# mapillary/OpenSfM

Measured on AMD Instinct MI355X. Metric: image-pairs matched/sec (+ BA LM-iters/sec, 5k cams / 500k pts), higher is better.
Workload: dtype i8 (exact int32 accumulate) + f64 RANSAC

## Files before the change

opensfm_amd/csrc/match.hip:

```cpp
#include <algorithm>
#include <cstdlib>
#include <type_traits>

#include "osfm_internal.h"

typedef int v4i __attribute__((ext_vector_type(4)));
typedef int v16i __attribute__((ext_vector_type(16)));

#ifdef OSFM_DBG_PHASES
__device__ unsigned long long g_phase[22];
#define OSFM_TICK(var) const unsigned long long var = wall_clock64();
#define OSFM_PHASE(i, t0, t1) if (threadIdx.x == 0) atomicAdd(&g_phase[i], (t1) - (t0));
extern "C" int osfm_dbg_phases(unsigned long long *out, int reset) {
  if (hipMemcpyFromSymbol(out, HIP_SYMBOL(g_phase), sizeof(g_phase)) != hipSuccess) return 1;
  if (reset) {
    unsigned long long z[22] = {};
    if (hipMemcpyToSymbol(HIP_SYMBOL(g_phase), z, sizeof(z)) != hipSuccess) return 1;
  }
  return 0;
}
#else
#define OSFM_TICK(var)
#define OSFM_PHASE(i, t0, t1)
#endif

namespace {

constexpr int kThreads = 256;
constexpr int kWaves = 4;
constexpr int kRT = 2;
constexpr int kNone = 0xFFFF;
constexpr int kCollisionD2 = 1 << 22;

__device__ __forceinline__ bool ratio_ok(int d1sq, int d2sq, double ratio) {
  if (ratio < 0.0) return (float)d1sq < (float)(-ratio) * (float)d2sq;
  const float f1 = sqrtf((float)d1sq), f2 = sqrtf((float)d2sq);
  return (double)f1 < ratio * (double)f2;
}

__device__ __forceinline__ long xcd_remap(long b, long n) {
  const long q = n >> 3, r = n & 7;
  const long xcd = b & 7, within = b >> 3;
  return (xcd < r ? xcd * (q + 1) : r * (q + 1) + (xcd - r) * q) + within;
}

struct MatchArgs {
  const int8_t *tiles;
  const int32_t *norms;
  const int32_t *hneg;
  const float *descf;
  const float *qerr;
  const int64_t *tile_off;
  const int32_t *counts;
  const int32_t *pairs;
  long n_pairs;
  double ratio;
  int symmetric;
  int query_second;
  int cap;
  int ncap;
  int32_t *out_counts;
  uint32_t *out_matches;
  int32_t *out_flags;
  long pad_tile;
  const uint32_t *bin;
  const float *seg;
  int32_t *tickets;
};
constexpr int kTicketStride = 32;

__device__ __forceinline__ void emit_matches(const MatchArgs &a, long p, int nC, const int *colBI,
                                             const unsigned short *rowres, int *misc, int tid, bool swap_halves) {
  const int lane = tid & 63, w = tid >> 6;
  int base = 0;
  for (int j0 = 0; j0 < nC; j0 += kThreads) {
    const int j = j0 + tid;
    bool m = false;
    int r = kNone;
    if (j < nC) {
      r = colBI[j];
      m = (r != kNone) && (!a.symmetric || rowres[r] == j);
    }
    const unsigned long long bal = __ballot(m);
    const int prefix = __popcll(bal & ((1ull << lane) - 1ull));
    if (lane == 0) misc[w] = __popcll(bal);
    __syncthreads();
    int woff = 0, total = 0;
#pragma unroll
    for (int w2 = 0; w2 < kWaves; ++w2) {
      const int cnt = misc[w2];
      woff += (w2 < w) ? cnt : 0;
      total += cnt;
    }
    if (m) {
      const int k = base + woff + prefix;
      if (k < a.cap) a.out_matches[p * a.cap + k] = swap_halves ? ((uint32_t)r | ((uint32_t)j << 16)) : ((uint32_t)j | ((uint32_t)r << 16));
    }
    base += total;
    __syncthreads();
  }
  if (tid == 0) a.out_counts[p] = base;
}

__device__ __forceinline__ int dot_rows8(const int8_t *tilesA, int rowA, const int8_t *tilesB, int rowB) {
  const int8_t *pa = tilesA + (long)(rowA >> 5) * OSFM_TILE_BYTES + (rowA & 31) * 16;
  const int8_t *pb = tilesB + (long)(rowB >> 5) * OSFM_TILE_BYTES + (rowB & 31) * 16;
  v4i av[8], bv[8];
#pragma unroll
  for (int q = 0; q < 8; ++q) {
    av[q] = *(const v4i *)(pa + q * 512);
    bv[q] = *(const v4i *)(pb + q * 512);
  }
  int s0 = 0, s1 = 0;
#pragma unroll
  for (int q = 0; q < 8; q += 2)
#pragma unroll
    for (int e = 0; e < 4; ++e) {
      s0 = __builtin_amdgcn_sdot4(av[q][e], bv[q][e], s0, false);
      s1 = __builtin_amdgcn_sdot4(av[q + 1][e], bv[q + 1][e], s1, false);
    }
  return s0 + s1;
}

template <class P>
__device__ __forceinline__ P *uniform_ptr(P *p) {
  const unsigned long long v = (unsigned long long)p;
  const unsigned lo = __builtin_amdgcn_readfirstlane((unsigned)v), hi = __builtin_amdgcn_readfirstlane((unsigned)(v >> 32));
  return (P *)(((unsigned long long)hi << 32) | lo);
}

__device__ __forceinline__ int wave_max(int v) {
#pragma unroll
  for (int m = 32; m >= 1; m >>= 1) v = max(v, __shfl_xor(v, m));
  return v;
}

__device__ __forceinline__ int row16_max(int x) {
  x = max(x, __builtin_amdgcn_update_dpp(x, x, 0xB1, 0xF, 0xF, false));
  x = max(x, __builtin_amdgcn_update_dpp(x, x, 0x4E, 0xF, 0xF, false));
  x = max(x, __builtin_amdgcn_update_dpp(x, x, 0x141, 0xF, 0xF, false));
  x = max(x, __builtin_amdgcn_update_dpp(x, x, 0x140, 0xF, 0xF, false));
  return x;
}

constexpr double kFqSlack = 8e-6;
__device__ __forceinline__ double fq_ratio(double ratio) { return ratio < 0.0 ? sqrt(-ratio) : ratio; }
__device__ __forceinline__ bool fq_surely_fails(int d0lo_sq, int d1hi_sq, double eps, double r) {
  const double D0lo = fmax(sqrt((double)max(d0lo_sq, 0)) - eps, 0.0) * (1.0 - kFqSlack);
  const double D1hi = (sqrt((double)max(d1hi_sq, 0)) + eps) * (1.0 + kFqSlack);
  return D0lo >= r * D1hi;
}
__device__ __forceinline__ bool fq_surely_passes(int d0hi_sq, int d1lo_sq, double eps, double r) {
  const double D0hi = (sqrt((double)max(d0hi_sq, 0)) + eps) * (1.0 + kFqSlack);
  const double D1lo = fmax(sqrt((double)max(d1lo_sq, 0)) - eps, 0.0) * (1.0 - kFqSlack);
  return D0hi < r * D1lo && D0hi < D1lo;
}
__device__ __forceinline__ float wave_minf(float v) {
#pragma unroll
  for (int m = 32; m >= 1; m >>= 1) v = fminf(v, __shfl_xor(v, m));
  return v;
}

constexpr int kCT4 = 8;
constexpr int kChunkCols4 = kCT4 * 32;
constexpr int kChunkBytes4 = kCT4 * OSFM_TILE_BYTES;

struct QueryPassShared {
  unsigned char *bbuf;
  int *hbuf;
};

template <bool GATHER, bool FQ, class Hooks>
__device__ __forceinline__ int query_pass(const QueryPassShared &sh, const int8_t *tilesQ, const int32_t *normQ, int nQ, int nslots,
                                          const unsigned short *qsel, const int8_t *tilesT, const int32_t *normT, const int32_t *hnegT,
                                          int nT, const int8_t *tiles_pad, const int32_t *hneg_pad, unsigned short *out, double ratio,
                                          int tid, const float *descQ, const float *descT, double eps, int *hit_word, int &any_hit,
                                          Hooks &&hooks) {
  asm volatile("" : "+v"(tid));
  asm volatile("" : "+s"(ratio));
  const int lane = tid & 63;
  const int w = __builtin_amdgcn_readfirstlane(tid >> 6);
  const int tT = (nT + 31) >> 5;
  const int tS = (nslots + 31) >> 5;
  const int nchunks = (tS + kCT4 - 1) / kCT4;
  const int nrb = (tT + kWaves * kRT - 1) / (kWaves * kRT);
  int flag = 0, hit = 0;

  auto dma_chunk = [&](int c) {
    unsigned char *dst = sh.bbuf + (c & 1) * kChunkBytes4;
#pragma unroll
    for (int q = 0; q < kCT4; ++q) {
      const int gt = c * kCT4 + q;
      const int8_t *src;
      if (GATHER) {
        const int slot = gt * 32 + (lane & 31);
        const int f = slot < nslots ? (int)qsel[slot] : 0;
        src = tilesQ + (long)(f >> 5) * OSFM_TILE_BYTES + w * 1024 + (lane >> 5) * 512 + (f & 31) * 16;
      } else {
        src = tilesQ + (long)(gt < tS ? gt : 0) * OSFM_TILE_BYTES + tid * 16;
      }
      __builtin_amdgcn_global_load_lds((const __attribute__((address_space(1))) void *)src,
                                       (__attribute__((address_space(3))) void *)(dst + q * OSFM_TILE_BYTES + w * 1024), 16, 0, 0);
    }
  };

  auto load_seeds = [&](int rb, int slot) {
    const int t = rb * (kWaves * kRT) + w * kRT;
    const int32_t *h0 = uniform_ptr((t < tT) ? hnegT + (long)t * 32 : hneg_pad);
    const int32_t *h1 = uniform_ptr((t + 1 < tT) ? hnegT + (long)(t + 1) * 32 : hneg_pad);
    const int32_t *hp = ((lane >> 5) ? h1 : h0) + (lane & 31);
    __builtin_amdgcn_global_load_lds((const __attribute__((address_space(1))) void *)hp,
                                     (__attribute__((address_space(3))) void *)(sh.hbuf + slot * 256 + w * 64), 4, 0, 0);
  };
  auto load_rows = [&](int rb, v4i (&af)[kRT][4], int rt) {
    const int t = rb * (kWaves * kRT) + w * kRT + rt;
    const auto *tp = (const __attribute__((address_space(1))) int8_t *)uniform_ptr((t < tT) ? tilesT + (long)t * OSFM_TILE_BYTES : tiles_pad);
#pragma unroll
    for (int ks = 0; ks < 4; ++ks) af[rt][ks] = *(const __attribute__((address_space(1))) v4i *)(tp + ks * 1024 + lane * 16);
  };
  auto load_targets = [&](int rb, v4i (&af)[kRT][4], int slot) {
    load_seeds(rb, slot);
    load_rows(rb, af, 0);
    load_rows(rb, af, 1);
  };
  v16i hn[kRT];
  auto read_seeds_rt = [&](int slot, int rt) {
#pragma unroll
    for (int g = 0; g < 4; ++g) {
      const v4i hv = *(const v4i *)(sh.hbuf + slot * 256 + w * 64 + rt * 32 + 8 * g + 4 * (lane >> 5));
      hn[rt][4 * g + 0] = hv[0];
      hn[rt][4 * g + 1] = hv[1];
      hn[rt][4 * g + 2] = hv[2];
      hn[rt][4 * g + 3] = hv[3];
    }
  };
  auto read_seeds = [&](int slot) {
    read_seeds_rt(slot, 0);
    read_seeds_rt(slot, 1);
  };

  int cb[kCT4], cs[kCT4], ci[kCT4];
  const unsigned char *bb = sh.bbuf;
  v4i bf[4];

#define OSFM_TREE_A(X, A, B)             \
  A = max(max(X[0], X[1]), X[2]);        \
  B = max(max(X[8], X[9]), X[10]);
#define OSFM_TREE_B(X, A, B)             \
  A = max(max(A, X[3]), X[4]);           \
  B = max(max(B, X[11]), X[12]);
#define OSFM_TREE_C(X, A, B)             \
  A = max(max(A, X[5]), X[6]);           \
  B = max(max(B, X[13]), X[14]);
// ... 25 lines not shown
        OSFM_TREE_A(C2, a0, b0)
        OSFM_TREE_B(C2, a0, b0)
        OSFM_TREE_C(C2, a0, b0)
        OSFM_TREE_D(C2, a0, b0, mp)
      } else {
        load_seeds(rbn, next_slot);
      }
      OSFM_PIN
      C2 = __builtin_amdgcn_mfma_i32_32x32x32_i8(af[1][0], bf[0], hn[1], 0, 0, 0);
      OSFM_PIN
      if (t == kCT4 - 1) {
        __builtin_amdgcn_s_waitcnt(0x0F70 | (2 * kRT * 4));
        read_seeds_rt(next_slot, 0);
      }
      bf[0] = *(const v4i *)(nb);
      if (t > 0) { OSFM_TREE_A(P2, a1, b1) }
      OSFM_PIN
      C1 = __builtin_amdgcn_mfma_i32_32x32x32_i8(af[0][1], bf[1], C1, 0, 0, 0);
      OSFM_PIN
      if (t > 0) { OSFM_TREE_B(P2, a1, b1) } else { load_rows(rbn, nxt, 0); }
      if (t == kCT4 - 1) read_seeds_rt(next_slot, 1);
      OSFM_PIN
      C2 = __builtin_amdgcn_mfma_i32_32x32x32_i8(af[1][1], bf[1], C2, 0, 0, 0);
      OSFM_PIN
      bf[1] = *(const v4i *)(nb + 1024);
      if (t > 0) { OSFM_TREE_C(P2, a1, b1) }
      OSFM_PIN
      C1 = __builtin_amdgcn_mfma_i32_32x32x32_i8(af[0][2], bf[2], C1, 0, 0, 0);
      OSFM_PIN
      if (t > 0) { OSFM_TREE_D(P2, a1, b1, m2) } else { load_rows(rbn, nxt, 1); }
      OSFM_PIN
      C2 = __builtin_amdgcn_mfma_i32_32x32x32_i8(af[1][2], bf[2], C2, 0, 0, 0);
      OSFM_PIN
      bf[2] = *(const v4i *)(nb + 2048);
      if (t > 0) {
        m2 = max(m2, mp);
        asm("v_med3_i32 %0, %1, %2, %3" : "=v"(cs[t - 1]) : "v"(cb[t - 1]), "v"(m2), "v"(cs[t - 1]));
      }
      OSFM_PIN
      C1 = __builtin_amdgcn_mfma_i32_32x32x32_i8(af[0][3], bf[3], C1, 0, 0, 0);
      OSFM_PIN
      if (t > 0)
        asm volatile("v_cmp_gt_i32 vcc, %1, %2\n\ts_nop 1\n\tv_cndmask_b32 %0, %0, %3, vcc" : "+v"(ci[t - 1]) : "v"(m2), "v"(cb[t - 1]), "v"(vrb) : "vcc");
      OSFM_PIN
      C2 = __builtin_amdgcn_mfma_i32_32x32x32_i8(af[1][3], bf[3], C2, 0, 0, 0);
      OSFM_PIN
      bf[3] = *(const v4i *)(nb + 3072);
      if (t > 0) cb[t - 1] = max(cb[t - 1], m2);
      OSFM_PIN
    }
    {
      v16i &Q1 = T[(2 * (kCT4 - 1)) % 3];
      v16i &Q2 = T[(2 * (kCT4 - 1) + 1) % 3];
      int a0, b0, a1, b1, m1, m2;
      OSFM_TREE_A(Q1, a0, b0)
      OSFM_TREE_B(Q1, a0, b0)
      OSFM_TREE_C(Q1, a0, b0)
      OSFM_TREE_D(Q1, a0, b0, m1)
      OSFM_TREE_A(Q2, a1, b1)
      OSFM_TREE_B(Q2, a1, b1)
      OSFM_TREE_C(Q2, a1, b1)
      OSFM_TREE_D(Q2, a1, b1, m2)
      m2 = max(m2, m1);
      asm("v_med3_i32 %0, %1, %2, %3" : "=v"(cs[kCT4 - 1]) : "v"(cb[kCT4 - 1]), "v"(m2), "v"(cs[kCT4 - 1]));
      ci[kCT4 - 1] = m2 > cb[kCT4 - 1] ? rb : ci[kCT4 - 1];
      cb[kCT4 - 1] = max(cb[kCT4 - 1], m2);
    }
  };

  auto load_norm = [&](int c) {
    const int slot = c * kChunkCols4 + tid;
    const int f = slot < nslots ? (GATHER ? (int)qsel[slot] : slot) : -1;
    return (f >= 0 && f < nQ) ? normQ[f] : OSFM_PAD_NORM;
  };
  dma_chunk(0);
  v4i afA[kRT][4], afB[kRT][4];
  load_targets(0, afA, 0);
  int myna_next = load_norm(0);
  hooks.cold_issue();
  __builtin_amdgcn_s_waitcnt(0x0F70);
  hooks.cold_done();
  read_seeds(0);
  int sidx = 0;

  for (int c = 0; c < nchunks; ++c) {
    const int myslot = c * kChunkCols4 + tid;
    const int myf = myslot < nslots ? (GATHER ? (int)qsel[myslot] : myslot) : -1;
    const int myna = myna_next;
    __builtin_amdgcn_s_waitcnt(0x0F70);
    __syncthreads();
    bb = sh.bbuf + (c & 1) * kChunkBytes4;
    const int t0 = kCT4 - min(kCT4, tS - c * kCT4);
#pragma unroll
    for (int ks = 0; ks < 4; ++ks) bf[ks] = *(const v4i *)(bb + ks * 1024 + lane * 16);
#pragma unroll
    for (int t = 0; t < kCT4; ++t) {
      cb[t] = INT_MIN;
      cs[t] = INT_MIN;
      ci[t] = 0;
    }

    auto one_step = [&](const v4i (&cur)[kRT][4], v4i (&nxt)[kRT][4], int rb) {
      const int rbn = (rb + 1 < nrb) ? rb + 1 : 0;
      const bool live = rb * (kWaves * kRT) + w * kRT < tT;
      const int nslot = (sidx + 1) & 1;
      if (live) {
        step(cur, nxt, rb, rbn, nslot, t0, bb - t0 * OSFM_TILE_BYTES);
      } else {
        load_targets(rbn, nxt, nslot);
        __builtin_amdgcn_s_waitcnt(0x0F70);
        read_seeds(nslot);
      }
      ++sidx;
    };
    OSFM_TICK(tk0)
    hooks.chunk(c);
    if (c + 1 < nchunks) dma_chunk(c + 1);
    int rb = 0;
    for (; rb + 1 < nrb; rb += 2) {
      one_step(afA, afB, rb);
      one_step(afB, afA, rb + 1);
    }
    if (rb < nrb) {
      one_step(afA, afB, rb);
#pragma unroll
      for (int rt = 0; rt < kRT; ++rt)
#pragma unroll
        for (int ks = 0; ks < 4; ++ks) afA[rt][ks] = afB[rt][ks];
    }

    OSFM_TICK(tk1)
    if (c + 1 < nchunks) myna_next = load_norm(c + 1);
    __syncthreads();
    OSFM_TICK(tk2)
    int *scr = (int *)(sh.bbuf + (c & 1) * kChunkBytes4);
    {
      const int part = w * 2 + (lane >> 5);
#pragma unroll
      for (int t = 0; t < kCT4; ++t) {
        const int qt = (t - t0) & (kCT4 - 1);
        scr[(part * 3 + 0) * kChunkCols4 + qt * 32 + (lane & 31)] = cb[t];
        scr[(part * 3 + 1) * kChunkCols4 + qt * 32 + (lane & 31)] = cs[t];
        scr[(part * 3 + 2) * kChunkCols4 + qt * 32 + (lane & 31)] = ci[t];
      }
    }
    __syncthreads();
    int b = INT_MIN, s2 = INT_MIN, id = 0;
#pragma unroll
    for (int part = 0; part < 2 * kWaves; ++part) {
      const int pb = scr[(part * 3 + 0) * kChunkCols4 + tid], ps = scr[(part * 3 + 1) * kChunkCols4 + tid];
      const int pi = scr[(part * 3 + 2) * kChunkCols4 + tid];
      s2 = max(max(s2, ps), min(b, pb));
      id = pb > b ? (pi * 8 + part) : id;
      b = max(b, pb);
    }
    __syncthreads();
    bool want = false;
    if (myf >= 0 && myf < nQ) {
      const int d1lo = max(myna - (2 * b + 1), 0), d2hi = myna - 2 * s2;
      if (FQ) {
        want = !fq_surely_fails(d1lo, d2hi, eps, fq_ratio(ratio));
      } else {
        if (d2hi >= kCollisionD2 && ratio >= 0.0) flag = 1;
        want = ratio_ok(d1lo, d2hi, ratio);
      }
#ifdef OSFM_DBG_NORECHECK
      want = false;
#endif
      if (!want) out[myf] = kNone;
    }
    unsigned long long pending = __ballot(want);
    unsigned long long redo = 0;
    OSFM_TICK(tk3)
#ifdef OSFM_DBG_PHASES
    if (tid == 0) atomicAdd(&g_phase[(GATHER ? 5 : 0) + 4], (unsigned long long)__popcll(pending));
#endif
    while (pending) {
      int srcs[4];
#pragma unroll
      for (int g = 0; g < 4; ++g) {
        srcs[g] = pending ? (int)__builtin_ctzll(pending) : -1;
        pending &= pending - 1;
      }
      const int g = lane >> 4, sl = lane & 15;
      const int src = g == 0 ? srcs[0] : g == 1 ? srcs[1] : g == 2 ? srcs[2] : srcs[3];
      const int ssrc = src < 0 ? 0 : src;
      const int qf = __shfl(myf, ssrc), qna = __shfl(myna, ssrc), qb = __shfl(b, ssrc), qs = __shfl(s2, ssrc), qid = __shfl(id, ssrc);
      const bool tie = (qs == qb);
      const int qrb = qid >> 3, qw = (qid >> 1) & 3, qh = qid & 1;
      const int row0 = (qrb * (kWaves * kRT) + qw * kRT) * 32 + (sl & 3) + 8 * (sl >> 2) + 4 * qh, row1 = row0 + 32;
      int k0 = INT_MIN, k1 = INT_MIN;
      if (src >= 0 && !tie) {
        const bool ok0 = row0 < nT, ok1 = row1 < nT;
        const int r0 = ok0 ? row0 : 0, r1 = ok1 ? row1 : 0;
        const int8_t *pa = tilesQ + (long)(qf >> 5) * OSFM_TILE_BYTES + (qf & 31) * 16;
        const int8_t *p0 = tilesT + (long)(r0 >> 5) * OSFM_TILE_BYTES + (r0 & 31) * 16;
        const int8_t *p1 = tilesT + (long)(r1 >> 5) * OSFM_TILE_BYTES + (r1 & 31) * 16;
        v4i av[8], bv0[8], bv1[8];
#pragma unroll
        for (int q = 0; q < 8; ++q) {
          av[q] = *(const v4i *)(pa + q * 512);
          bv0[q] = *(const v4i *)(p0 + q * 512);
          bv1[q] = *(const v4i *)(p1 + q * 512);
        }
        const int n0 = normT[r0], n1 = normT[r1];
        int s0 = 0, s1 = 0;
#pragma unroll
        for (int q = 0; q < 8; ++q)
#pragma unroll
          for (int e = 0; e < 4; ++e) {
            s0 = __builtin_amdgcn_sdot4(av[q][e], bv0[q][e], s0, false);
            s1 = __builtin_amdgcn_sdot4(av[q][e], bv1[q][e], s1, false);
          }
        if (ok0) k0 = (2 * s0 - n0) * 32 + (31 - sl);
        if (ok1) k1 = (2 * s1 - n1) * 32 + (15 - sl);
      }
      const int kmax = row16_max(max(k0, k1));
      const int ksec = row16_max(k0 == kmax ? k1 : (k1 == kmax ? k0 : max(k0, k1)));
      if (src >= 0) {
        bool full = tie;
        int win = kNone;
        if (!tie) {
          const int m1 = kmax >> 5, ord = 31 - (kmax & 31);
          const int jwin = (qrb * (kWaves * kRT) + qw * kRT + (ord >> 4)) * 32 + (ord & 3) + 8 * ((ord & 15) >> 2) + 4 * qh;
          const int m2 = ksec >> 5;
          const int sa = max(m2, 2 * qs), sb = max(m2, 2 * qs + 1);
          if (FQ) {
            const double r = fq_ratio(ratio);
            if (fq_surely_passes(qna - m1, qna - sb, eps, r))
              win = jwin;
            else if (!fq_surely_fails(qna - m1, qna - sa, eps, r))
              full = true;
          } else {
            const bool ra = ratio_ok(qna - m1, qna - sa, ratio), rbb = ratio_ok(qna - m1, qna - sb, ratio);
            if (ra == rbb)
              win = ra ? jwin : kNone;
            else
              full = true;
          }
        }
        if (sl == 0 && !full) out[qf] = (unsigned short)win;
        hit |= (!full && win != kNone);
        redo |= (full && sl == 0) ? (1ull << src) : 0ull;
      }
    }
    OSFM_TICK(tk4)
    OSFM_PHASE((GATHER ? 5 : 0) + 0, tk0, tk1)
    OSFM_PHASE((GATHER ? 5 : 0) + 1, tk1, tk2)
    OSFM_PHASE((GATHER ? 5 : 0) + 2, tk2, tk3)
    OSFM_PHASE((GATHER ? 5 : 0) + 3, tk3, tk4)
    {
      unsigned lo = (unsigned)redo, hi = (unsigned)(redo >> 32);
#pragma unroll
      for (int m = 32; m >= 16; m >>= 1) {
        lo |= (unsigned)__shfl_xor((int)lo, m);
        hi |= (unsigned)__shfl_xor((int)hi, m);
      }
      redo = ((unsigned long long)(unsigned)__builtin_amdgcn_readfirstlane((int)hi) << 32) | (unsigned)__builtin_amdgcn_readfirstlane((int)lo);
    }
    if (FQ) flag += __popcll(redo);
    while (FQ && redo) {
      const int src = __builtin_ctzll(redo);
      redo &= redo - 1;
      const int qf = __shfl(myf, src), qna = __shfl(myna, src), qs2 = __shfl(s2, src);
      const double T = (sqrt((double)max(qna - 2 * qs2, 0)) + 2.0 * eps) * (1.0 + 4.0 * kFqSlack) + 1e-6;
      const double T2 = T * T;
      const int vthr = T2 >= 2.0e9 ? INT_MIN : qna - (int)T2 - 1;
      const float *qrow = descQ + (long)qf * OSFM_DESC_DIM;
      float bd0 = INFINITY, bd1 = INFINITY;
      int bi0 = INT_MAX;
      for (int i = lane; i < nT; i += 64) {
        const int v = 2 * dot_rows8(tilesQ, qf, tilesT, i) - normT[i];
        if (v >= vthr) {
          const float sq = l2sqr_rows_f32(qrow, descT + (long)i * OSFM_DESC_DIM);
          const float d = ratio < 0.0 ? sq : sqrtf(sq);
          if (d < bd1) {
            if (bd0 > d) {
              bd1 = bd0;
              bd0 = d;
              bi0 = i;
            } else {
              bd1 = d;
            }
          }
        }
      }
      const float m = wave_minf(bd0);
      const int jwin = -wave_max(bd0 == m ? -bi0 : INT_MIN);
      const float sec = wave_minf(bi0 == jwin ? bd1 : bd0);
      const bool ok = ratio < 0.0 ? (m < (float)(-ratio) * sec) : ((double)m < ratio * (double)sec);
      if (lane == 0) out[qf] = (unsigned short)(ok ? jwin : kNone);
      hit |= ok;
    }
    while (!FQ && redo) {
      const int src = __builtin_ctzll(redo);
      redo &= redo - 1;
      const int qf = __shfl(myf, src), qna = __shfl(myna, src);
      int lv = INT_MIN, lj = INT_MAX, ls = INT_MIN;
      for (int i = lane; i < nT; i += 64) {
        const int v = 2 * dot_rows8(tilesQ, qf, tilesT, i) - normT[i];
        ls = max(ls, min(lv, v));
        if (v > lv) {
          lv = v;
          lj = i;
        }
      }
      const int m1 = wave_max(lv);
      const int jwin = -wave_max(lv == m1 ? -lj : INT_MIN);
      const int m2 = wave_max(lj == jwin ? ls : lv);
      const bool ok = ratio_ok(qna - m1, qna - m2, ratio);
      if (lane == 0) out[qf] = (unsigned short)(ok ? jwin : kNone);
      hit |= ok;
    }
  }
  if (hit) *hit_word = 1;
  __syncthreads();
  any_hit = *hit_word;
  return flag;
}

struct PairRange {
  long first;
  int len;
};
__device__ __forceinline__ PairRange pair_range(long n_pairs, int x) {
  const long q = n_pairs >> 3, r = n_pairs & 7;
  return PairRange{x < r ? x * (q + 1) : r * (q + 1) + (x - r) * q, (int)(q + (x < r ? 1 : 0))};
}
__device__ __forceinline__ int draw_pair(const MatchArgs &a, int xcd, int *hdr, bool have, int t) {
  for (int k = hdr[8]; k < 8; ++k) {
    const int x = (xcd + k) & 7;
    const PairRange r = pair_range(a.n_pairs, x);
    if (!have) t = atomicAdd(a.tickets + x * kTicketStride, 1);
    have = false;
    if (t < r.len) {
      hdr[8] = k;
      return (int)(r.first + t);
    }
  }
  hdr[8] = 8;
  return -1;
}
__device__ __forceinline__ void finish_pair_header(const MatchArgs &a, int *hdr) {
  const int img1 = hdr[1], img2 = hdr[2];
  const int n1 = a.counts[img1], n2 = a.counts[img2];
  const int o1 = (int)a.tile_off[img1], o2 = (int)a.tile_off[img2];
  hdr[3] = n1;
  hdr[4] = n2;
  hdr[5] = o1;
  hdr[6] = o2;
  hdr[7] = 1;
}
__device__ __forceinline__ void fetch_pair_header(const MatchArgs &a, int xcd, int *hdr) {
  const int p = draw_pair(a, xcd, hdr, false, 0);
  hdr[0] = p;
  hdr[7] = 1;
  if (p >= 0) {
    const int img1 = a.pairs[2 * (long)p], img2 = a.pairs[2 * (long)p + 1];
    hdr[1] = img1;
    hdr[2] = img2;
    finish_pair_header(a, hdr);
  }
}
struct NextPairFetch {
  const MatchArgs &a;
  int xcd;
  int *hdr;
  int tid;
  int t;
  __device__ __forceinline__ void cold_issue() {
    if (tid == 0) {
      const int k = hdr[8];
      t = k < 8 ? atomicAdd(a.tickets + ((xcd + k) & 7) * kTicketStride, 1) : 0;
    }
  }
  __device__ __forceinline__ void cold_done() {
    if (tid == 0) {
      hdr[0] = draw_pair(a, xcd, hdr, hdr[8] < 8, t);
      hdr[7] = 0;
    }
  }
  __device__ __forceinline__ void chunk(int c) {
    if (c > 1 || __builtin_amdgcn_readfirstlane(tid >> 6) != 0) return;
    const int pn = __builtin_amdgcn_readfirstlane(hdr[0]);
    if (pn < 0) return;
    if (c == 0) {
      if (tid < 2)
        __builtin_amdgcn_global_load_lds((const __attribute__((address_space(1))) void *)(a.pairs + 2 * (long)pn + tid),
                                         (__attribute__((address_space(3))) void *)(hdr + 1), 4, 0, 0);
    } else if (tid < 4) {
      const int img = hdr[1 + (tid & 1)];
      const int32_t *src = tid < 2 ? a.counts + img : (const int32_t *)(a.tile_off + img);
      __builtin_amdgcn_global_load_lds((const __attribute__((address_space(1))) void *)src,
                                       (__attribute__((address_space(3))) void *)(hdr + 3), 4, 0, 0);
      if (tid == 0) hdr[7] = 1;
    }
  }
};
struct NoFetch {
  __device__ __forceinline__ void cold_issue() {}
  __device__ __forceinline__ void cold_done() {}
  __device__ __forceinline__ void chunk(int) {}
};

__device__ __forceinline__ int fresh_tid(int wave) {
  int t = wave * 64 + (int)__builtin_amdgcn_mbcnt_hi(~0u, __builtin_amdgcn_mbcnt_lo(~0u, 0u));
  asm volatile("" : "+v"(t));
  return t;
}

template <bool FQ>
__global__ void __launch_bounds__(kThreads, 2) match_fused_kernel(MatchArgs a) {
  extern __shared__ __attribute__((aligned(16))) unsigned char smem[];
  QueryPassShared sh;
  sh.bbuf = smem;
  sh.hbuf = (int *)(smem + 2 * kChunkBytes4);
  int *misc = (int *)(smem + 2 * kChunkBytes4) + 2 * kChunkCols4;
  int *hdr = misc + 16;
  unsigned short *resA = (unsigned short *)(hdr + 16);
  unsigned short *resB = resA + a.ncap;
  unsigned short *cand = resB + a.ncap;

  const int xcd = blockIdx.x & 7;
  const int8_t *tiles_pad = a.tiles + a.pad_tile * OSFM_TILE_BYTES;
  const int32_t *hneg_pad = a.hneg + a.pad_tile * 32;
  OSFM_TICK(tw0)
#ifdef OSFM_DBG_PHASES
  unsigned long long t_prev = tw0;
#endif
  const int wave = __builtin_amdgcn_readfirstlane(threadIdx.x >> 6);
  if (threadIdx.x == 0) {
    hdr[8] = 0;
    fetch_pair_header(a, xcd, hdr);
  }
  __syncthreads();
  for (;;) {
  const int tid = fresh_tid(wave);
  const long p = __builtin_amdgcn_readfirstlane(hdr[0]);
  if (p < 0) break;
  if (__builtin_amdgcn_readfirstlane(hdr[7]) == 0) {
    __syncthreads();
    if (tid == 0) finish_pair_header(a, hdr);
    __syncthreads();
  }
  const int img1 = __builtin_amdgcn_readfirstlane(hdr[1]), img2 = __builtin_amdgcn_readfirstlane(hdr[2]);
  const int n1 = __builtin_amdgcn_readfirstlane(hdr[3]), n2 = __builtin_amdgcn_readfirstlane(hdr[4]);
  const long off1 = __builtin_amdgcn_readfirstlane(hdr[5]), off2 = __builtin_amdgcn_readfirstlane(hdr[6]);
  if (tid == 0) {
    misc[8] = 0;
    misc[9] = 0;
    misc[10] = 0;
  }
  __syncthreads();
  if (n1 < 2 || n2 < 2) {
    if (tid == 0) {
      a.out_counts[p] = 0;
      a.out_flags[p] = 0;
      fetch_pair_header(a, xcd, hdr);
    }
    __syncthreads();
#ifdef OSFM_DBG_PHASES
    {
      OSFM_TICK(te)
      OSFM_PHASE(19, t_prev, te)
      if (threadIdx.x == 0) atomicAdd(&g_phase[20], 1ull);
      t_prev = te;
    }
#endif
    continue;
  }
  const bool rows_second = a.symmetric || a.query_second;
  const int imgA = rows_second ? img2 : img1, imgB = rows_second ? img1 : img2;
  const int nA = rows_second ? n2 : n1, nB = rows_second ? n1 : n2;
  const long offA = rows_second ? off2 : off1, offB = rows_second ? off1 : off2;
  const int8_t *tilesA = a.tiles + offA * OSFM_TILE_BYTES;
  const int8_t *tilesB = a.tiles + offB * OSFM_TILE_BYTES;
  const int32_t *normA = a.norms + offA * 32;
  const int32_t *normB = a.norms + offB * 32;
  const int32_t *hnegA = a.hneg + offA * 32;
  const int32_t *hnegB = a.hneg + offB * 32;
  OSFM_TICK(tq0)
  const float *descA = FQ ? a.descf + offA * (long)(32 * OSFM_DESC_DIM) : nullptr;
  const float *descB = FQ ? a.descf + offB * (long)(32 * OSFM_DESC_DIM) : nullptr;
  const double eps = FQ ? (double)a.qerr[imgA] + (double)a.qerr[imgB] : 0.0;
  int any = 0;
  auto flush_flag = [&](int f) {
    if (FQ) {
      if ((fresh_tid(wave) & 63) == 0 && f) atomicAdd(&misc[8], f);
    } else if (f) {
      misc[8] = 1;
    }
  };
  int flag = query_pass<false, FQ>(sh, tilesA, normA, nA, nA, nullptr, tilesB, normB, hnegB, nB, tiles_pad, hneg_pad, resA, a.ratio, fresh_tid(wave),
                                   descA, descB, eps, misc + 9, any, NextPairFetch{a, xcd, hdr, fresh_tid(wave), 0});
  OSFM_TICK(tq1)
  OSFM_PHASE(10, tq0, tq1)
  if (a.symmetric && any) {
    const int tid = fresh_tid(wave), lane = tid & 63, w = tid >> 6;
    for (int j = tid; j < nB; j += kThreads) resB[j] = kNone;
    __syncthreads();
    for (int q = tid; q < nA; q += kThreads) {
      const int b = resA[q];
      if (b != kNone) resB[b] = 0;
    }
// ... 250 lines not shown
  const int nC = a.counts[imgC], nR = a.counts[imgR];
  if (nC < 2 || nR < 2) {
    if (tid == 0) a.out_counts[p] = 0;
    return;
  }
  const float *descC = a.descf + a.tile_off[imgC] * kFloatTileFloats;
  const float *descR = a.descf + a.tile_off[imgR] * kFloatTileFloats;
  float_direction(descC, nC, descR, nR, a.ratio, tid, stage, colBI, nullptr);
  if (a.symmetric) float_direction(descR, nR, descC, nC, a.ratio, tid, stage, nullptr, rowres);
  __syncthreads();
  emit_matches(a, p, nC, colBI, rowres, misc, tid, qs);
}

constexpr int kHamStageRows = 256;

__device__ void hamming_direction(const uint32_t *binQ, int nQ, const uint32_t *binT, int nT, double ratio, int tid, uint32_t *stage, int *res_int,
                                  unsigned short *res_u16) {
  for (int q0 = 0; q0 < nQ; q0 += kThreads) {
    const int q = q0 + tid;
    const bool live = q < nQ;
    uint4 qa[4];
#pragma unroll
    for (int k = 0; k < 4; ++k) qa[k] = live ? *(const uint4 *)(binQ + (size_t)q * 16 + 4 * k) : make_uint4(0u, 0u, 0u, 0u);
    int bd0 = 0x7fffffff, bd1 = 0x7fffffff, bi0 = kNone;
    for (int t0 = 0; t0 < nT; t0 += kHamStageRows) {
      const int nt = min(kHamStageRows, nT - t0);
      __syncthreads();
      for (int k = tid; k < nt * 4; k += kThreads) *(uint4 *)(stage + 4 * k) = *(const uint4 *)(binT + (size_t)t0 * 16 + 4 * k);
      __syncthreads();
      for (int t = 0; t < nt; ++t) {
        const uint4 *b = (const uint4 *)(stage + t * 16);
        int d = 0;
#pragma unroll
        for (int k = 0; k < 4; ++k) {
          const uint4 c = b[k];
          d += __popc(qa[k].x ^ c.x) + __popc(qa[k].y ^ c.y) + __popc(qa[k].z ^ c.z) + __popc(qa[k].w ^ c.w);
        }
        if (d < bd1) {
          if (bd0 > d) {
            bd1 = bd0;
            bd0 = d;
            bi0 = t0 + t;
          } else {
            bd1 = d;
          }
        }
      }
    }
    if (live) {
      const bool ok = (double)(float)bd0 < ratio * (double)(float)bd1;
      const int v = ok ? bi0 : kNone;
      if (res_int) res_int[q] = v;
      if (res_u16) res_u16[q] = (unsigned short)v;
    }
  }
}

__global__ void __launch_bounds__(kThreads) match_hamming_kernel(MatchArgs a) {
  extern __shared__ __attribute__((aligned(16))) unsigned char smem[];
  uint32_t *stage = (uint32_t *)smem;
  int *colBI = (int *)(stage + kHamStageRows * 16);
  unsigned short *rowres = (unsigned short *)(colBI + a.ncap);
  int *misc = (int *)(rowres + a.ncap);
  const int tid = threadIdx.x;
  const long p = blockIdx.x;
  if (tid == 0 && a.out_flags) a.out_flags[p] = 0;
  const bool qs = !a.symmetric && a.query_second;
  const int imgC = a.pairs[2 * p + (qs ? 1 : 0)], imgR = a.pairs[2 * p + (qs ? 0 : 1)];
  const int nC = a.counts[imgC], nR = a.counts[imgR];
  if (nC < 2 || nR < 2) {
    if (tid == 0) a.out_counts[p] = 0;
    return;
  }
  const uint32_t *binC = a.bin + a.tile_off[imgC] * (32 * 16);
  const uint32_t *binR = a.bin + a.tile_off[imgR] * (32 * 16);
  hamming_direction(binC, nC, binR, nR, a.ratio, tid, stage, colBI, nullptr);
  if (a.symmetric) hamming_direction(binR, nR, binC, nC, a.ratio, tid, stage, nullptr, rowres);
  __syncthreads();
  emit_matches(a, p, nC, colBI, rowres, misc, tid, qs);
}

}

size_t osfm_match_lds_bytes(int ncap) { return (size_t)2 * kChunkBytes4 + 2 * kChunkCols4 * 4 + 128 + (size_t)ncap * 6; }

static int ensure_kernel_attributes(int device) {
  static OsfmPerDeviceOnce once;
  return once.run(device, []() -> int {
    OSFM_HIP(hipFuncSetAttribute((const void *)match_fused_kernel<false>, hipFuncAttributeMaxDynamicSharedMemorySize, 160 * 1024));
    OSFM_HIP(hipFuncSetAttribute((const void *)match_fused_kernel<true>, hipFuncAttributeMaxDynamicSharedMemorySize, 160 * 1024));
    OSFM_HIP(hipFuncSetAttribute((const void *)match_exact_kernel, hipFuncAttributeMaxDynamicSharedMemorySize, 160 * 1024));
    OSFM_HIP(hipFuncSetAttribute((const void *)match_float_kernel, hipFuncAttributeMaxDynamicSharedMemorySize, 160 * 1024));
    OSFM_HIP(hipFuncSetAttribute((const void *)match_hamming_kernel, hipFuncAttributeMaxDynamicSharedMemorySize, 160 * 1024));
    return OSFM_OK;
  });
}

int osfm_launch_match(osfm_ctx *ctx, const osfm_store *store, const int32_t *d_pairs, int64_t n_pairs,
                      double ratio, int symmetric, int squared_ratio, int cap, int32_t *d_counts, uint32_t *d_matches,
                      int32_t *d_flags, bool exact_kernel, hipStream_t stream) {
  if (n_pairs == 0) return OSFM_OK;
  MatchArgs a;
  a.tiles = store->d_tiles;
  a.norms = store->d_norms;
  a.hneg = store->d_hneg;
  a.descf = store->d_descf;
  a.qerr = store->d_qerr;
  a.seg = store->d_seg;
  a.bin = store->d_bin;
  a.tile_off = store->d_tile_off;
  a.counts = store->d_counts;
  a.pairs = d_pairs;
  a.n_pairs = n_pairs;
  a.ratio = squared_ratio ? -(double)(float)(ratio * ratio) : ratio;
  a.symmetric = symmetric;
  a.query_second = squared_ratio && !symmetric;
  a.cap = cap;
  a.ncap = ((store->max_count + 127) / 128) * 128;
  if (a.ncap < 128) a.ncap = 128;
  a.out_counts = d_counts;
  a.out_matches = d_matches;
  a.out_flags = d_flags;
  a.pad_tile = store->tile_off[store->n_images];
  a.tickets = nullptr;
  OSFM_REQUIRE(a.ncap <= OSFM_MAX_FEATURES, OSFM_E_UNSUPPORTED, "more than %d features in an image", OSFM_MAX_FEATURES);
  OSFM_REQUIRE(n_pairs < (1ll << 31), OSFM_E_INVALID, "too many pairs in one launch");
  OSFM_TRY(ensure_kernel_attributes(ctx->device));
  const bool fused = !store->is_binary && !store->d_seg && !exact_kernel && (!store->is_float || store->quantised);
  unsigned resident = 0;
  if (fused) {
    OSFM_REQUIRE(a.pad_tile < (1ll << 31), OSFM_E_UNSUPPORTED, "too many tiles in the store");
    OSFM_REQUIRE(ctx->num_cus > 0, OSFM_E_INVALID, "the context knows no compute units");
    if (!ctx->d_match_tickets) OSFM_HIP(hipMalloc(&ctx->d_match_tickets, 8 * kTicketStride * sizeof(int32_t)));
    OSFM_HIP(hipMemsetAsync(ctx->d_match_tickets, 0, 8 * kTicketStride * sizeof(int32_t), stream));
    a.tickets = (int32_t *)ctx->d_match_tickets;
    resident = (unsigned)std::min<int64_t>(n_pairs, 2 * (int64_t)ctx->num_cus);
  }
  if (store->is_binary) {
    if (squared_ratio) a.ratio = ratio * ratio;
    if (exact_kernel && d_flags != nullptr) return OSFM_OK;
    const size_t lds = (size_t)kHamStageRows * 64 + (size_t)a.ncap * 6 + 64;
    hipLaunchKernelGGL(match_hamming_kernel, dim3((unsigned)n_pairs), dim3(kThreads), lds, stream, a);
  } else if (store->d_seg) {
    if (exact_kernel && d_flags != nullptr) return OSFM_OK;
    if (d_flags) OSFM_HIP(hipMemsetAsync(d_flags, 0, (size_t)n_pairs * sizeof(int32_t), stream));
    const size_t lds = (size_t)a.ncap * 6 + 64;
    hipLaunchKernelGGL(match_exact_kernel, dim3((unsigned)n_pairs), dim3(kThreads), lds, stream, a, 0);
  } else if (store->is_float) {
    if (exact_kernel && d_flags != nullptr) return OSFM_OK;
    if (!exact_kernel && store->quantised) {
      hipLaunchKernelGGL(match_fused_kernel<true>, dim3(resident), dim3(kThreads), osfm_match_lds_bytes(a.ncap), stream, a);
    } else {
      if (d_flags) OSFM_HIP(hipMemsetAsync(d_flags, 0, (size_t)n_pairs * sizeof(int32_t), stream));
      const size_t lds = (size_t)kFloatTileFloats * sizeof(float) + (size_t)a.ncap * 6 + 64;
      hipLaunchKernelGGL(match_float_kernel, dim3((unsigned)n_pairs), dim3(kThreads), lds, stream, a);
    }
  } else if (!exact_kernel) {
    hipLaunchKernelGGL(match_fused_kernel<false>, dim3(resident), dim3(kThreads), osfm_match_lds_bytes(a.ncap), stream, a);
  } else {
    const size_t lds = (size_t)a.ncap * 6 + 64;
    hipLaunchKernelGGL(match_exact_kernel, dim3((unsigned)n_pairs), dim3(kThreads), lds, stream, a, d_flags != nullptr ? 1 : 0);
  }
  OSFM_HIP(hipGetLastError());
  return OSFM_OK;
}
```

Baseline: 2.799 million.

## Batch ratio-test recheck candidates across chunks in LDS and spread over all waves

Instead of each wave immediately rechecking its own ambiguous queries after every chunk, candidates are appended to a block-wide LDS pending queue (with overflow into the scratch area) and flushed only once enough accumulate or at the last chunk. The flush spreads rounds of four candidates across all waves, double-buffers the gathers of target rows and query words, and broadcasts query words with ds_swizzle instead of loading them per lane. One barrier is dropped, and full fallback scans are deferred to a second pass marked by a redo bit. The intent is better load balance and latency hiding for the sparse recheck work, at the cost of added LDS, extra complexity, and longer liveness of pending entries.

After: 2.795 million. About the same (-0.1%).

```diff
diff --git a/opensfm_amd/csrc/match.hip b/opensfm_amd/csrc/match.hip
--- a/opensfm_amd/csrc/match.hip
+++ b/opensfm_amd/csrc/match.hip
@@ -8,13 +8,13 @@
 typedef int v16i __attribute__((ext_vector_type(16)));
 
 #ifdef OSFM_DBG_PHASES
-__device__ unsigned long long g_phase[22];
+__device__ unsigned long long g_phase[26];
 #define OSFM_TICK(var) const unsigned long long var = wall_clock64();
 #define OSFM_PHASE(i, t0, t1) if (threadIdx.x == 0) atomicAdd(&g_phase[i], (t1) - (t0));
 extern "C" int osfm_dbg_phases(unsigned long long *out, int reset) {
   if (hipMemcpyFromSymbol(out, HIP_SYMBOL(g_phase), sizeof(g_phase)) != hipSuccess) return 1;
   if (reset) {
-    unsigned long long z[22] = {};
+    unsigned long long z[26] = {};
     if (hipMemcpyToSymbol(HIP_SYMBOL(g_phase), z, sizeof(z)) != hipSuccess) return 1;
   }
   return 0;
@@ -168,7 +168,13 @@
 struct QueryPassShared {
   unsigned char *bbuf;
   int *hbuf;
+  int *pend;
+  int *pend_n;
 };
+constexpr int kPendFlush = 16;
+constexpr int kPendCap = kPendFlush;
+constexpr int kPendTie = 1 << 30;
+constexpr int kPendRedo = (int)0x80000000u;
 
 template <bool GATHER, bool FQ, class Hooks>
 __device__ __forceinline__ int query_pass(const QueryPassShared &sh, const int8_t *tilesQ, const int32_t *normQ, int nQ, int nslots,
@@ -360,6 +366,8 @@
   hooks.cold_done();
   read_seeds(0);
   int sidx = 0;
+  if (tid == 0) *sh.pend_n = 0;
+  int pend_done = 0;
 
   for (int c = 0; c < nchunks; ++c) {
     const int myslot = c * kChunkCols4 + tid;
@@ -400,6 +408,7 @@
       one_step(afB, afA, rb + 1);
     }
     if (rb < nrb) {
+      asm volatile("v_nop");
       one_step(afA, afB, rb);
 #pragma unroll
       for (int rt = 0; rt < kRT; ++rt)
@@ -432,7 +441,6 @@
       id = pb > b ? (pi * 8 + part) : id;
       b = max(b, pb);
     }
-    __syncthreads();
     bool want = false;
     if (myf >= 0 && myf < nQ) {
       const int d1lo = max(myna - (2 * b + 1), 0), d2hi = myna - 2 * s2;
@@ -447,149 +455,263 @@
 #endif
       if (!want) out[myf] = kNone;
     }
-    unsigned long long pending = __ballot(want);
-    unsigned long long redo = 0;
+    int *ovf = scr + 2 * kWaves * 3 * kChunkCols4;
+    {
+      const unsigned long long wb = __ballot(want);
+#ifdef OSFM_DBG_PHASES
+      if (tid == 0) atomicAdd(&g_phase[(GATHER ? 5 : 0) + 4], (unsigned long long)__popcll(wb));
+#endif
+      if (wb) {
+        int base = 0;
+        if (lane == 0) base = atomicAdd(sh.pend_n, (int)__popcll(wb));
+        base = __builtin_amdgcn_readfirstlane(base) - pend_done;
+        if (want) {
+          const int e = base + (int)__builtin_amdgcn_mbcnt_hi((unsigned)(wb >> 32), __builtin_amdgcn_mbcnt_lo((unsigned)wb, 0u));
+          int *ent = e < kPendCap ? sh.pend + 2 * e : ovf + 2 * (e - kPendCap);
+          ent[0] = myf | (id << 16) | (s2 == b ? kPendTie : 0);
+          ent[1] = s2;
+        }
+      }
+    }
+    __syncthreads();
     OSFM_TICK(tk3)
+    int npend;
+    {
+      auto *pn = (volatile __attribute__((address_space(3))) int *)sh.pend_n;
+      asm volatile("" : "+s"(pn));
+      npend = __builtin_amdgcn_readfirstlane(*pn) - pend_done;
+    }
+    if (npend > 0 && (npend >= kPendFlush || c + 1 == nchunks)) {
+      const int rounds = (npend + 3) >> 2;
 #ifdef OSFM_DBG_PHASES
-    if (tid == 0) atomicAdd(&g_phase[(GATHER ? 5 : 0) + 4], (unsigned long long)__popcll(pending));
+      if (tid == 0) {
+        atomicAdd(&g_phase[(GATHER ? 24 : 22)], 1ull);
+        atomicAdd(&g_phase[(GATHER ? 25 : 23)], (unsigned long long)rounds);
+      }
 #endif
-    while (pending) {
-      int srcs[4];
-#pragma unroll
-      for (int g = 0; g < 4; ++g) {
-        srcs[g] = pending ? (int)__builtin_ctzll(pending) : -1;
-        pending &= pending - 1;
-      }
-      const int g = lane >> 4, sl = lane & 15;
-      const int src = g == 0 ? srcs[0] : g == 1 ? srcs[1] : g == 2 ? srcs[2] : srcs[3];
-      const int ssrc = src < 0 ? 0 : src;
-      const int qf = __shfl(myf, ssrc), qna = __shfl(myna, ssrc), qb = __shfl(b, ssrc), qs = __shfl(s2, ssrc), qid = __shfl(id, ssrc);
-      const bool tie = (qs == qb);
-      const int qrb = qid >> 3, qw = (qid >> 1) & 3, qh = qid & 1;
-      const int row0 = (qrb * (kWaves * kRT) + qw * kRT) * 32 + (sl & 3) + 8 * (sl >> 2) + 4 * qh, row1 = row0 + 32;
-      int k0 = INT_MIN, k1 = INT_MIN;
-      if (src >= 0 && !tie) {
-        const bool ok0 = row0 < nT, ok1 = row1 < nT;
-        const int r0 = ok0 ? row0 : 0, r1 = ok1 ? row1 : 0;
-        const int8_t *pa = tilesQ + (long)(qf >> 5) * OSFM_TILE_BYTES + (qf & 31) * 16;
-        const int8_t *p0 = tilesT + (long)(r0 >> 5) * OSFM_TILE_BYTES + (r0 & 31) * 16;
-        const int8_t *p1 = tilesT + (long)(r1 >> 5) * OSFM_TILE_BYTES + (r1 & 31) * 16;
-        v4i av[8], bv0[8], bv1[8];
+      int fl = (int)__builtin_amdgcn_mbcnt_hi(~0u, __builtin_amdgcn_mbcnt_lo(~0u, 0u));
+      asm volatile("" : "+v"(fl));
+      const int g = fl >> 4, sl = fl & 15;
+      struct ReexamRound {
+        v4i t0[8], t1[8];
+        int qx, qy;
+        int n0, n1, qna;
+      };
+      typedef __attribute__((address_space(3))) int lds_int;
+      lds_int *pend3 = (lds_int *)sh.pend, *ovf3 = (lds_int *)ovf;
+      asm volatile("" : "+s"(pend3), "+s"(ovf3));
+      auto entry = [&](int e) { return e < kPendCap ? pend3 + 2 * e : ovf3 + 2 * (e - kPendCap); };
+      struct ReexamAddr {
+        const int8_t *pa, *p0, *p1;
+        const int32_t *n0, *n1, *na;
+      };
+      auto locate = [&](int r) {
+        const bool real = r < rounds;
+        const int e = 4 * r + g;
+        const int x = entry(real && e < npend ? e : 0)[0];
+        const int qf = x & 0xFFFF, qid = (x >> 16) & 0x7FF;
+        const int qrb = qid >> 3, qw = (qid >> 1) & 3, qh = qid & 1;
+        const int row0 = (qrb * (kWaves * kRT) + qw * kRT) * 32 + (sl & 3) + 8 * (sl >> 2) + 4 * qh, row1 = row0 + 32;
+        const int r0 = row0 < nT ? row0 : 0, r1 = row1 < nT ? row1 : 0;
+        ReexamAddr A;
+        A.pa = real ? tilesQ + (long)(qf >> 5) * OSFM_TILE_BYTES + (qf & 31) * 16 + (sl >> 1) * 512 + (sl & 1) * 8 : tiles_pad;
+        A.p0 = real ? tilesT + (long)(r0 >> 5) * OSFM_TILE_BYTES + (r0 & 31) * 16 : tiles_pad;
+        A.p1 = real ? tilesT + (long)(r1 >> 5) * OSFM_TILE_BYTES + (r1 & 31) * 16 : tiles_pad;
+        A.n0 = real ? normT + r0 : hneg_pad;
+        A.n1 = real ? normT + r1 : hneg_pad;
+        A.na = real ? normQ + qf : hneg_pad;
+        return A;
+      };
+      auto gather = [&](ReexamRound &S, const ReexamAddr &A) {
 #pragma unroll
         for (int q = 0; q < 8; ++q) {
-          av[q] = *(const v4i *)(pa + q * 512);
-          bv0[q] = *(const v4i *)(p0 + q * 512);
-          bv1[q] = *(const v4i *)(p1 + q * 512);
+          S.t0[q] = *(const v4i *)(A.p0 + q * 512);
+          S.t1[q] = *(const v4i *)(A.p1 + q * 512);
         }
-        const int n0 = normT[r0], n1 = normT[r1];
+        S.qx = ((const int *)A.pa)[0];
+        S.qy = ((const int *)A.pa)[1];
+        S.n0 = *A.n0;
+        S.n1 = *A.n1;
+        S.qna = *A.na;
+      };
+      auto issue = [&](ReexamRound &S, int r) { gather(S, locate(r)); };
+#define OSFM_ROWLANE(v, k) __builtin_amdgcn_ds_swizzle((v), 0x10 | ((k) << 5))
+#define OSFM_REEXAM_WORDS(S, q)                                                                    \
+  const int a##q##0 = OSFM_ROWLANE(S.qx, 2 * (q)), a##q##1 = OSFM_ROWLANE(S.qy, 2 * (q)),         \
+            a##q##2 = OSFM_ROWLANE(S.qx, 2 * (q) + 1), a##q##3 = OSFM_ROWLANE(S.qy, 2 * (q) + 1);
+#define OSFM_REEXAM_DOTS(S, q)                                   \
+  s0 = __builtin_amdgcn_sdot4(a##q##0, S.t0[q][0], s0, false);   \
+  s1 = __builtin_amdgcn_sdot4(a##q##0, S.t1[q][0], s1, false);   \
+  s0 = __builtin_amdgcn_sdot4(a##q##1, S.t0[q][1], s0, false);   \
+  s1 = __builtin_amdgcn_sdot4(a##q##1, S.t1[q][1], s1, false);   \
+  s0 = __builtin_amdgcn_sdot4(a##q##2, S.t0[q][2], s0, false);   \
+  s1 = __builtin_amdgcn_sdot4(a##q##2, S.t1[q][2], s1, false);   \
+  s0 = __builtin_amdgcn_sdot4(a##q##3, S.t0[q][3], s0, false);   \
+  s1 = __builtin_amdgcn_sdot4(a##q##3, S.t1[q][3], s1, false);
+      auto redo_all = [&](int qf, int qna, int qs2) {
+        if (FQ) {
+          const double T = (sqrt((double)max(qna - 2 * qs2, 0)) + 2.0 * eps) * (1.0 + 4.0 * kFqSlack) + 1e-6;
+          const double T2 = T * T;
+          const int vthr = T2 >= 2.0e9 ? INT_MIN : qna - (int)T2 - 1;
+          const float *qrow = descQ + (long)qf * OSFM_DESC_DIM;
+          float bd0 = INFINITY, bd1 = INFINITY;
+          int bi0 = INT_MAX;
+          for (int i = fl; i < nT; i += 64) {
+            const int v = 2 * dot_rows8(tilesQ, qf, tilesT, i) - normT[i];
+            if (v >= vthr) {
+              const float sq = l2sqr_rows_f32(qrow, descT + (long)i * OSFM_DESC_DIM);
+              const float d = ratio < 0.0 ? sq : sqrtf(sq);
+              if (d < bd1) {
+                if (bd0 > d) {
+                  bd1 = bd0;
+                  bd0 = d;
+                  bi0 = i;
+                } else {
+                  bd1 = d;
+                }
+              }
+            }
+          }
+          const float m = wave_minf(bd0);
+          const int jwin = -wave_max(bd0 == m ? -bi0 : INT_MIN);
+          const float sec = wave_minf(bi0 == jwin ? bd1 : bd0);
+          const bool ok = ratio < 0.0 ? (m < (float)(-ratio) * sec) : ((double)m < ratio * (double)sec);
+          if (fl == 0) out[qf] = (unsigned short)(ok ? jwin : kNone);
+          hit |= ok;
+        } else {
+          int lv = INT_MIN, lj = INT_MAX, ls = INT_MIN;
+          for (int i = fl; i < nT; i += 64) {
+            const int v = 2 * dot_rows8(tilesQ, qf, tilesT, i) - normT[i];
+            ls = max(ls, min(lv, v));
+            if (v > lv) {
+              lv = v;
+              lj = i;
+            }
+          }
+          const int m1 = wave_max(lv);
+          const int jwin = -wave_max(lv == m1 ? -lj : INT_MIN);
+          const int m2 = wave_max(lj == jwin ? ls : lv);
+          const bool ok = ratio_ok(qna - m1, qna - m2, ratio);
+          if (fl == 0) out[qf] = (unsigned short)(ok ? jwin : kNone);
+          hit |= ok;
+        }
+      };
+      bool any_redo = false;
+      auto evaluate = [&](ReexamRound &S, int r) {
         int s0 = 0, s1 = 0;
-#pragma unroll
-        for (int q = 0; q < 8; ++q)
-#pragma unroll
-          for (int e = 0; e < 4; ++e) {
-            s0 = __builtin_amdgcn_sdot4(av[q][e], bv0[q][e], s0, false);
-            s1 = __builtin_amdgcn_sdot4(av[q][e], bv1[q][e], s1, false);
+        OSFM_PIN
+        OSFM_REEXAM_WORDS(S, 0)
+        OSFM_REEXAM_WORDS(S, 1)
+        OSFM_REEXAM_WORDS(S, 2)
+        OSFM_REEXAM_WORDS(S, 3)
+        OSFM_REEXAM_WORDS(S, 4)
+        OSFM_REEXAM_WORDS(S, 5)
+        OSFM_REEXAM_WORDS(S, 6)
+        OSFM_REEXAM_WORDS(S, 7)
+        OSFM_PIN
+        __builtin_amdgcn_s_waitcnt(0xC07F);
+        OSFM_PIN
+        OSFM_REEXAM_DOTS(S, 0)
+        OSFM_REEXAM_DOTS(S, 1)
+        OSFM_REEXAM_DOTS(S, 2)
+        OSFM_REEXAM_DOTS(S, 3)
+        OSFM_REEXAM_DOTS(S, 4)
+        OSFM_REEXAM_DOTS(S, 5)
+        OSFM_REEXAM_DOTS(S, 6)
+        OSFM_REEXAM_DOTS(S, 7)
+        asm volatile("" : "+v"(s0), "+v"(s1));
+        const int e = 4 * r + g;
+        const bool have = e < npend;
+        lds_int *ent = entry(have ? e : 0);
+        const int x = ent[0], qs = ent[1];
+        const int qf = x & 0xFFFF, qid = (x >> 16) & 0x7FF, qna = S.qna;
+        const bool tie = (x & kPendTie) != 0;
+        const int qrb = qid >> 3, qw = (qid >> 1) & 3, qh = qid & 1;
+        const int row0 = (qrb * (kWaves * kRT) + qw * kRT) * 32 + (sl & 3) + 8 * (sl >> 2) + 4 * qh, row1 = row0 + 32;
+        int k0 = INT_MIN, k1 = INT_MIN;
+        if (have && !tie) {
+          if (row0 < nT) k0 = (2 * s0 - S.n0) * 32 + (31 - sl);
+          if (row1 < nT) k1 = (2 * s1 - S.n1) * 32 + (15 - sl);
+        }
+        const int kmax = row16_max(max(k0, k1));
+        const int ksec = row16_max(k0 == kmax ? k1 : (k1 == kmax ? k0 : max(k0, k1)));
+        bool full = false;
+        if (have) {
+          full = tie;
+          int win = kNone;
+          if (!tie) {
+            const int m1 = kmax >> 5, ord = 31 - (kmax & 31);
+            const int jwin = (qrb * (kWaves * kRT) + qw * kRT + (ord >> 4)) * 32 + (ord & 3) + 8 * ((ord & 15) >> 2) + 4 * qh;
+            const int m2 = ksec >> 5;
+            const int sa = max(m2, 2 * qs), sb = max(m2, 2 * qs + 1);
+            if (FQ) {
+              const double r = fq_ratio(ratio);
+              if (fq_surely_passes(qna - m1, qna - sb, eps, r))
+                win = jwin;
+              else if (!fq_surely_fails(qna - m1, qna - sa, eps, r))
+                full = true;
+            } else {
+              const bool ra = ratio_ok(qna - m1, qna - sa, ratio), rbb = ratio_ok(qna - m1, qna - sb, ratio);
+              if (ra == rbb)
+                win = ra ? jwin : kNone;
+              else
+                full = true;
+            }
           }
-        if (ok0) k0 = (2 * s0 - n0) * 32 + (31 - sl);
-        if (ok1) k1 = (2 * s1 - n1) * 32 + (15 - sl);
-      }
-      const int kmax = row16_max(max(k0, k1));
-      const int ksec = row16_max(k0 == kmax ? k1 : (k1 == kmax ? k0 : max(k0, k1)));
-      if (src >= 0) {
-        bool full = tie;
-        int win = kNone;
-        if (!tie) {
-          const int m1 = kmax >> 5, ord = 31 - (kmax & 31);
-          const int jwin = (qrb * (kWaves * kRT) + qw * kRT + (ord >> 4)) * 32 + (ord & 3) + 8 * ((ord & 15) >> 2) + 4 * qh;
-          const int m2 = ksec >> 5;
-          const int sa = max(m2, 2 * qs), sb = max(m2, 2 * qs + 1);
-          if (FQ) {
-            const double r = fq_ratio(ratio);
-            if (fq_surely_passes(qna - m1, qna - sb, eps, r))
-              win = jwin;
-            else if (!fq_surely_fails(qna - m1, qna - sa, eps, r))
-              full = true;
-          } else {
-            const bool ra = ratio_ok(qna - m1, qna - sa, ratio), rbb = ratio_ok(qna - m1, qna - sb, ratio);
-            if (ra == rbb)
-              win = ra ? jwin : kNone;
-            else
-              full = true;
+          if (sl == 0 && !full) out[qf] = (unsigned short)win;
+          hit |= (!full && win != kNone);
+        }
+        if (full && sl == 0) ent[0] = x | kPendRedo;
+        any_redo |= __ballot(full) != 0ull;
+      };
+      int r = w;
+      if (r < rounds) {
+        ReexamRound S0, S1;
+        int r1 = r + kWaves;
+        {
+          const ReexamAddr A0 = locate(r), A1 = locate(r1);
+          __builtin_amdgcn_sched_barrier(0);
+          gather(S0, A0);
+          gather(S1, A1);
+        }
+        evaluate(S0, r);
+        while (r1 < rounds) {
+          r = r1 + kWaves;
+          issue(S0, r);
+          evaluate(S1, r1);
+          if (r >= rounds) break;
+          r1 = r + kWaves;
+          issue(S1, r1);
+          evaluate(S0, r);
+        }
+      }
+      if (any_redo) {
+        for (r = w; r < rounds; r += kWaves) {
+          const int e = 4 * r + g;
+          const bool have = e < npend;
+          const lds_int *ent = entry(have ? e : 0);
+          const int x = ent[0], qs = ent[1];
+          unsigned long long redo = __ballot(have && sl == 0 && (x & kPendRedo));
+          if (FQ) flag += __popcll(redo);
+          while (redo) {
+            const int src = __builtin_ctzll(redo);
+            redo &= redo - 1;
+            const int qf = __shfl(x, src) & 0xFFFF;
+            redo_all(qf, normQ[qf], __shfl(qs, src));
           }
         }
-        if (sl == 0 && !full) out[qf] = (unsigned short)win;
-        hit |= (!full && win != kNone);
-        redo |= (full && sl == 0) ? (1ull << src) : 0ull;
-      }
+      }
+#undef OSFM_REEXAM_WORDS
+#undef OSFM_REEXAM_DOTS
+#undef OSFM_ROWLANE
+      pend_done += npend;
+      read_seeds(sidx & 1);
     }
     OSFM_TICK(tk4)
     OSFM_PHASE((GATHER ? 5 : 0) + 0, tk0, tk1)
     OSFM_PHASE((GATHER ? 5 : 0) + 1, tk1, tk2)
     OSFM_PHASE((GATHER ? 5 : 0) + 2, tk2, tk3)
     OSFM_PHASE((GATHER ? 5 : 0) + 3, tk3, tk4)
-    {
-      unsigned lo = (unsigned)redo, hi = (unsigned)(redo >> 32);
-#pragma unroll
-      for (int m = 32; m >= 16; m >>= 1) {
-        lo |= (unsigned)__shfl_xor((int)lo, m);
-        hi |= (unsigned)__shfl_xor((int)hi, m);
-      }
-      redo = ((unsigned long long)(unsigned)__builtin_amdgcn_readfirstlane((int)hi) << 32) | (unsigned)__builtin_amdgcn_readfirstlane((int)lo);
-    }
-    if (FQ) flag += __popcll(redo);
-    while (FQ && redo) {
-      const int src = __builtin_ctzll(redo);
-      redo &= redo - 1;
-      const int qf = __shfl(myf, src), qna = __shfl(myna, src), qs2 = __shfl(s2, src);
-      const double T = (sqrt((double)max(qna - 2 * qs2, 0)) + 2.0 * eps) * (1.0 + 4.0 * kFqSlack) + 1e-6;
-      const double T2 = T * T;
-      const int vthr = T2 >= 2.0e9 ? INT_MIN : qna - (int)T2 - 1;
-      const float *qrow = descQ + (long)qf * OSFM_DESC_DIM;
-      float bd0 = INFINITY, bd1 = INFINITY;
-      int bi0 = INT_MAX;
-      for (int i = lane; i < nT; i += 64) {
-        const int v = 2 * dot_rows8(tilesQ, qf, tilesT, i) - normT[i];
-        if (v >= vthr) {
-          const float sq = l2sqr_rows_f32(qrow, descT + (long)i * OSFM_DESC_DIM);
-          const float d = ratio < 0.0 ? sq : sqrtf(sq);
-          if (d < bd1) {
-            if (bd0 > d) {
-              bd1 = bd0;
-              bd0 = d;
-              bi0 = i;
-            } else {
-              bd1 = d;
-            }
-          }
-        }
-      }
-      const float m = wave_minf(bd0);
-      const int jwin = -wave_max(bd0 == m ? -bi0 : INT_MIN);
-      const float sec = wave_minf(bi0 == jwin ? bd1 : bd0);
-      const bool ok = ratio < 0.0 ? (m < (float)(-ratio) * sec) : ((double)m < ratio * (double)sec);
-      if (lane == 0) out[qf] = (unsigned short)(ok ? jwin : kNone);
-      hit |= ok;
-    }
-    while (!FQ && redo) {
-      const int src = __builtin_ctzll(redo);
-      redo &= redo - 1;
-      const int qf = __shfl(myf, src), qna = __shfl(myna, src);
-      int lv = INT_MIN, lj = INT_MAX, ls = INT_MIN;
-      for (int i = lane; i < nT; i += 64) {
-        const int v = 2 * dot_rows8(tilesQ, qf, tilesT, i) - normT[i];
-        ls = max(ls, min(lv, v));
-        if (v > lv) {
-          lv = v;
-          lj = i;
-        }
-      }
-      const int m1 = wave_max(lv);
-      const int jwin = -wave_max(lv == m1 ? -lj : INT_MIN);
-      const int m2 = wave_max(lj == jwin ? ls : lv);
-      const bool ok = ratio_ok(qna - m1, qna - m2, ratio);
-      if (lane == 0) out[qf] = (unsigned short)(ok ? jwin : kNone);
-      hit |= ok;
-    }
   }
   if (hit) *hit_word = 1;
   __syncthreads();
@@ -698,6 +820,8 @@
   unsigned short *resA = (unsigned short *)(hdr + 16);
   unsigned short *resB = resA + a.ncap;
   unsigned short *cand = resB + a.ncap;
+  sh.pend = (int *)(cand + a.ncap);
+  sh.pend_n = misc + 11;
 
   const int xcd = blockIdx.x & 7;
   const int8_t *tiles_pad = a.tiles + a.pad_tile * OSFM_TILE_BYTES;
@@ -1114,7 +1238,9 @@
 
 }
 
-size_t osfm_match_lds_bytes(int ncap) { return (size_t)2 * kChunkBytes4 + 2 * kChunkCols4 * 4 + 128 + (size_t)ncap * 6; }
+size_t osfm_match_lds_bytes(int ncap) {
+  return (size_t)2 * kChunkBytes4 + 2 * kChunkCols4 * 4 + 128 + (size_t)ncap * 6 + (size_t)kPendCap * 8;
+}
 
 static int ensure_kernel_attributes(int device) {
   static OsfmPerDeviceOnce once;
```
